# TAMS-Group/bio_ik

Measured on AMD Instinct MI355X. Metric: IK solves/sec (pop=128, 7-DOF PoseGoal batch), higher is better.
Workload: dtype f64

## Files before the change

bio_ik_amd/csrc/bioik_kernels.h:

```cpp
#pragma once
#include <type_traits>

#include "bioik_device.h"


#ifndef BIOIK_CANDIDATE_BOUND
#define BIOIK_CANDIDATE_BOUND BIOIK_SINCOS_DOMAIN
#endif
#ifndef BIOIK_COOP_WALKS
#define BIOIK_COOP_WALKS 1
#endif

struct LdsLayout {
    int seed, par, pop, sol, prefix, state, clip, xcol, slots, g_first, g_stride, total;
    int xn, gv, frames, tips, delta, base, grad, red, sec, order, bc;
    int xm, xp, dv, fc;
    int fitp;
    int help;
};
BIOIK_HD LdsLayout make_layout(int n_ops, int V, int P, int T, int n_slots, int nthreads, int lambda, int has_secondary, int child_cols = 1,
                               int groups = 1, int slot_sets = 1, int fit_park = 0, int fc_in_pop = 0, int helped = 0, int bounded = 0) {
    LdsLayout L;
    const int m = n_ops > 0 ? n_ops : 1;
    int o = 0;
// ... 62 lines not shown
};
BIOIK_DEV bool cand_better(double f, int pos, double of, int opos) { return (f < of) || (f == of && pos < opos); }

BIOIK_DEV void top2_insert(double& b1f, int& b1p, double& b2f, int& b2p, double f, int pos) {
    const bool w1 = cand_better(f, pos, b1f, b1p), w2 = cand_better(f, pos, b2f, b2p);
    b2f = w1 ? b1f : (w2 ? f : b2f);
    b2p = w1 ? b1p : (w2 ? pos : b2p);
    b1f = w1 ? f : b1f;
    b1p = w1 ? pos : b1p;
}
BIOIK_DEV void top2_merge(double& b1f, int& b1p, double& b2f, int& b2p, double o1f, int o1p, double o2f, int o2p) {
    const bool w1 = cand_better(o1f, o1p, b1f, b1p);
    const bool k2 = cand_better(b1f, b1p, o2f, o2p);
    const bool w2 = cand_better(o1f, o1p, b2f, b2p);
    const double n2f = w1 ? (k2 ? b1f : o2f) : (w2 ? o1f : b2f);
    const int n2p = w1 ? (k2 ? b1p : o2p) : (w2 ? o1p : b2p);
    b1f = w1 ? o1f : b1f;
    b1p = w1 ? o1p : b1p;
    b2f = n2f, b2p = n2p;
}
BIOIK_DEV double wave_min_f64(double v) {
    v = fmin(v, p_quad_xor<1>(v));
    v = fmin(v, p_quad_xor<2>(v));
    v = fmin(v, p_row_mirror<1>(v));
    v = fmin(v, p_row_mirror<0>(v));
    return fmin(fmin(p_read_lane(v, 0), p_read_lane(v, 16)), fmin(p_read_lane(v, 32), p_read_lane(v, 48)));
}
BIOIK_DEV int imin(int a, int b) { return a < b ? a : b; }
BIOIK_DEV int wave_min_i32(int v) {
    v = imin(v, p_quad_xor<1>(v));
    v = imin(v, p_quad_xor<2>(v));
    v = imin(v, p_row_mirror<1>(v));
    v = imin(v, p_row_mirror<0>(v));
    return imin(imin(p_read_lane(v, 0), p_read_lane(v, 16)), imin(p_read_lane(v, 32), p_read_lane(v, 48)));
}
BIOIK_DEV int wave_argmin(double f, int pos, double& mf, int& mp) {
    mf = wave_min_f64(f);
    const unsigned long long tied = p_ballot(f == mf);
    int lane;
    if ((tied & (tied - 1ull)) == 0ull) {
        lane = __builtin_ctzll(tied);
    } else {
        const int pm = wave_min_i32(f == mf ? pos : 0x7fffffff);
        lane = __builtin_ctzll(p_ballot(f == mf && pos == pm));
    }
    mp = p_read_lane(pos, lane);
    return lane;
}
BIOIK_DEV void top2_wave64_minima(double& b1f, int& b1p, double& b2f, int& b2p) {
    double w1f, w2f;
    int w1p, w2p;
    const int l1 = wave_argmin(b1f, b1p, w1f, w1p);
    const bool mine = (p_tid() & 63) == l1;
    wave_argmin(mine ? b2f : b1f, mine ? b2p : b1p, w2f, w2p);
    b1f = w1f, b1p = w1p, b2f = w2f, b2p = w2p;
}
BIOIK_DEV void top2_wave(double& b1f, int& b1p, double& b2f, int& b2p, int G) {
#if !defined(BIOIK_TOP2_BUTTERFLY)
    if (G >= 64) {
        top2_wave64_minima(b1f, b1p, b2f, b2p);
        return;
    }
#endif
#pragma unroll
    for (int m = 32; m >= 16; m >>= 1) {
        if (m >= G) continue;
        double o1f = p_shfl_xor(b1f, m), o2f = p_shfl_xor(b2f, m);
        int o1p = p_shfl_xor(b1p, m), o2p = p_shfl_xor(b2p, m);
        top2_merge(b1f, b1p, b2f, b2p, o1f, o1p, o2f, o2p);
    }
#define TOP2_DPP_STEP(MOVE)                                          \
    {                                                                \
        const double o1f = MOVE(b1f), o2f = MOVE(b2f);               \
        const int o1p = MOVE(b1p), o2p = MOVE(b2p);                  \
        top2_merge(b1f, b1p, b2f, b2p, o1f, o1p, o2f, o2p);          \
    }
    TOP2_DPP_STEP(p_row_mirror<0>)
    TOP2_DPP_STEP(p_row_mirror<1>)
    TOP2_DPP_STEP(p_quad_xor<2>)
    TOP2_DPP_STEP(p_quad_xor<1>)
#undef TOP2_DPP_STEP
}
template <int E>
BIOIK_DEV void sort_pairs_in_registers(double (&f)[E], int (&c)[E], int gtid, int G) {
    const int n = G * E;
    for (int k = 2; k <= n; k <<= 1) {
        const bool ascending = ((gtid * E) & k) == 0;
        for (int j = k >> 1; j >= E; j >>= 1) {
            const int d = j / E;
            const bool keep_low = ((gtid & d) == 0) == ascending;
#pragma unroll
            for (int i = 0; i < E; i++) {
                const double of = p_shfl_xor(f[i], d);
                const int oc = p_shfl_xor(c[i], d);
                const bool mine_after = (f[i] > of) || (f[i] == of && c[i] > oc);
                const bool take = mine_after == keep_low;
                f[i] = take ? of : f[i], c[i] = take ? oc : c[i];
            }
        }
#pragma unroll
        for (int j = E >> 1; j > 0; j >>= 1) {
            if (j >= k) continue;
#pragma unroll
            for (int i = 0; i < E; i++) {
                if (i & j) continue;
                const int i2 = i | j;
                const bool asc = k >= E ? ascending : ((i & k) == 0);
                const bool a_after_b = (f[i] > f[i2]) || (f[i] == f[i2] && c[i] > c[i2]);
                const bool swap = a_after_b == asc;
                const double fa = f[i], fb = f[i2];
                const int ca = c[i], cb = c[i2];
                f[i] = swap ? fb : fa, f[i2] = swap ? fa : fb, c[i] = swap ? cb : ca, c[i2] = swap ? ca : cb;
            }
        }
    }
}
template <int E>
BIOIK_DEV void sort_keys_in_registers(unsigned long long (&key)[E], int gtid, int G) {
    const int n = G * E;
    for (int k = 2; k <= n; k <<= 1) {
        const bool ascending = ((gtid * E) & k) == 0;
        for (int j = k >> 1; j >= E; j >>= 1) {
            const int d = j / E;
            const bool keep_low = ((gtid & d) == 0) == ascending;
#pragma unroll
            for (int i = 0; i < E; i++) {
                const unsigned long long other = p_shfl_xor(key[i], d);
                key[i] = ((key[i] > other) == keep_low) ? other : key[i];
            }
        }
#pragma unroll
        for (int j = E >> 1; j > 0; j >>= 1) {
            if (j >= k) continue;
#pragma unroll
            for (int i = 0; i < E; i++) {
                if (i & j) continue;
                const int i2 = i | j;
                const bool asc = k >= E ? ascending : ((i & k) == 0);
                const unsigned long long a = key[i], b = key[i2];
                const bool swap = (a > b) == asc;
                key[i] = swap ? b : a, key[i2] = swap ? a : b;
            }
        }
    }
}
BIOIK_DEV unsigned long long half_min_u64(unsigned long long k) {
    unsigned long long o = p_shfl_xor(k, 16);
    k = o < k ? o : k;
    o = p_row_mirror<0>(k), k = o < k ? o : k;
    o = p_row_mirror<1>(k), k = o < k ? o : k;
    o = p_quad_xor<2>(k), k = o < k ? o : k;
    o = p_quad_xor<1>(k), k = o < k ? o : k;
    return k;
}
BIOIK_DEV unsigned long long group_min_u64(unsigned long long k, int G) {
    if (G >= 64) {
        const unsigned long long o = p_shfl_xor(k, 32);
        k = o < k ? o : k;
    }
    return half_min_u64(k);
}
template <int E>
BIOIK_DEV unsigned long long select_threshold(const unsigned long long (&key)[E], int n_mine, int k, int G, unsigned long long gmask, bool& found) {
    unsigned long long lo = ~0ull, nhi = ~0ull;
#pragma unroll
    for (int i = 0; i < E; i++)
        if (i < n_mine) lo = key[i] < lo ? key[i] : lo, nhi = ~key[i] < nhi ? ~key[i] : nhi;
    lo = group_min_u64(lo, G);
    unsigned long long hi = ~group_min_u64(nhi, G);
    unsigned long long T = hi;
    bool done = false;
    for (int round = 0; round < 66; round++) {
        const unsigned long long mid = lo + ((hi - lo) >> 1);
        int cnt = 0;
#pragma unroll
        for (int i = 0; i < E; i++) cnt += p_popc64(p_ballot(key[i] <= mid) & gmask);
        if (!done) {
            if (cnt == k) T = mid, done = true;
            else if (cnt < k) lo = mid + 1ull;
            else hi = mid;
        }
        if (p_ballot(!done) == 0ull) break;
    }
    found = done;
    return T;
}
BIOIK_DEV unsigned long long sort_key(double f, int index, int drop) {
    unsigned long long b;
    __builtin_memcpy(&b, &f, 8);
    return (b & ~((1ull << drop) - 1ull)) | (unsigned long long)index;
}
BIOIK_DEV void group_sync(int G) {
    if (G > 64) p_barrier(); else p_wave_sync();
}
BIOIK_DEV void top2_xwave(double& b1f, int& b1p, double& b2f, int& b2p, double* s_red, int gtid, int G) {
    const int nw = G >> 6;
    if (G > 64) {
        if ((gtid & 63) == 0) {
            double* d = s_red + 4 * (gtid >> 6);
            d[0] = b1f, d[1] = (double)b1p, d[2] = b2f, d[3] = (double)b2p;
        }
        p_barrier();
        b1f = b2f = P_INF;
        b1p = b2p = 0x7fffffff;
        for (int w = 0; w < nw; w++) {
            const double* d = s_red + 4 * w;
            for (int i = 0; i < 2; i++) {
                double of = d[2 * i];
                int op = (int)d[2 * i + 1];
                top2_insert(b1f, b1p, b2f, b2p, of, op);
            }
        }
        p_barrier();
    }
}

template <int COOP = 0, class PB>
BIOIK_NOINLINE void build_approximator(PB pb, XV x, double* slots, double* s_frames, double* s_tips, double* s_delta, double* s_base, int gtid, int G,
                                       const double* prefix = nullptr) {
    const int n_ops = pb->n_ops, T = pb->T;
    if (gtid < 64) {
        auto publish = [&](int t, const F7& f) {
            if (gtid == 0) f7_store(s_tips + t * 7, f);
        };
        if (COOP == 0) fk_walk(pb, x, slots, gtid == 0 ? s_frames : nullptr, publish, prefix);
        else if (G >= 64) fk_walk<64>(pb, x, slots, gtid == 0 ? s_frames : nullptr, publish, prefix);
        else fk_walk<32>(pb, x, slots, gtid == 0 ? s_frames : nullptr, publish, prefix);
    }
    for (int k = gtid; k < n_ops; k += G) s_base[k] = x(k);
    group_sync(G);
    for (int t = 0; t < T; t++)
        for (int k = gtid; k < n_ops; k += G) {
            double o[7];
            approximator_entry(pb, t, k, s_frames, s_tips, o, s_base, prefix);
            double* d = s_delta + ((size_t)t * n_ops + k) * 7;
            for (int c = 0; c < 7; c++) d[c] = o[c];
        }
    group_sync(G);
}

struct SelectArgs {
    int islands, V;
    int sync, pad;
    uint64_t n;
    const double* isl_solutions;
    const double* isl_fitness;
    const int32_t* isl_success;
    const int32_t* isl_steps;
    double* solutions;
    double* fitness;
    int32_t* success;
    int32_t* steps;
};
BIOIK_DEV void select_body(const SelectArgs& a, uint64_t q) {
    if (q >= a.n) return;
    int best = 0;
    double best_fit = BIOIK_DBL_MAX;
    int least_steps = 0x7fffffff;
    if (a.sync)
        for (int i = 0; i < a.islands; i++) {
            uint64_t u = q * (uint64_t)a.islands + i;
            if (p_load_device(a.isl_success + u) && p_load_device(a.isl_steps + u) < least_steps) least_steps = p_load_device(a.isl_steps + u);
        }
    for (int i = 0; i < a.islands; i++) {
        uint64_t u = q * (uint64_t)a.islands + i;
        if (p_load_device(a.isl_success + u) && (!a.sync || p_load_device(a.isl_steps + u) == least_steps) && p_load_device(a.isl_fitness + u) < best_fit) best_fit = p_load_device(a.isl_fitness + u), best = i;
    }
    if (best_fit == BIOIK_DBL_MAX) {
        for (int i = 0; i < a.islands; i++) {
            uint64_t u = q * (uint64_t)a.islands + i;
            if (p_load_device(a.isl_fitness + u) < best_fit) best_fit = p_load_device(a.isl_fitness + u), best = i;
        }
    }
    uint64_t u = q * (uint64_t)a.islands + best;
    for (int v = 0; v < a.V; v++) a.solutions[q * a.V + v] = p_load_device(a.isl_solutions + u * a.V + v);
    a.fitness[q] = best_fit;
    a.success[q] = p_load_device(a.isl_success + u);
    a.steps[q] = p_load_device(a.isl_steps + u);
}

BIOIK_DEV void select_coop(const SelectArgs& a, uint64_t q, int lane) {
    const uint64_t u0 = q * (uint64_t)a.islands;
    int least = 0x7fffffff;
    if (a.sync) {
        for (int i = lane; i < a.islands; i += 64) {
            const int st = p_load_device(a.isl_steps + u0 + i);
            if (p_load_device(a.isl_success + u0 + i) && st < least) least = st;
        }
        for (int m = 32; m >= 1; m >>= 1) {
            const int o = p_shfl_xor(least, m);
            least = o < least ? o : least;
        }
    }
    double bf = BIOIK_DBL_MAX, af = BIOIK_DBL_MAX;
    int bi = 0x7fffffff, ai = 0x7fffffff;
    for (int i = lane; i < a.islands; i += 64) {
        const double f = p_load_device(a.isl_fitness + u0 + i);
        const bool counts = p_load_device(a.isl_success + u0 + i) && (!a.sync || p_load_device(a.isl_steps + u0 + i) == least);
        if (counts && f < bf) bf = f, bi = i;
        if (f < af) af = f, ai = i;
    }
    for (int m = 32; m >= 1; m >>= 1) {
        const double obf = p_shfl_xor(bf, m), oaf = p_shfl_xor(af, m);
        const int obi = p_shfl_xor(bi, m), oai = p_shfl_xor(ai, m);
        if (obf < bf || (obf == bf && obi < bi)) bf = obf, bi = obi;
        if (oaf < af || (oaf == af && oai < ai)) af = oaf, ai = oai;
// ... 720 lines not shown
template <class Frame>
BIOIK_DEV void solve_walks(Frame& F, SpeciesState& S, double*& popS, int rank_it, int step, int gen, uint32_t ctr1, int n_eval, double& b1f, int& b1p, double& b2f, int& b2p) {
    BIOIK_FRAME_NAMES(F);
    auto rank_now = [&]() { return F.rank_now(rank_it); };
    unsigned int& gen_count = F.gen_count;
    bool& lost = F.lost;
    auto rendezvous_lost = [&]() { F.rendezvous_lost(); };
    BIOIK_LANE_SCOPE;
    const double* cb = popS + S.cur * BF;
    const double *p0g = cb, *p0d = cb + M, *p1d = cb + 3 * M;
    const uint32_t gctr = (uint32_t)step * 16u + (uint32_t)gen;
    const bool stored = !columnless && n_cols * G >= lambda && (LEAN || pb->n_quat == 0);
    auto offer = [&](double f, int pos) { top2_insert(b1f, b1p, b2f, b2p, f, pos); };
    auto coarse_parked = [&](int gt) {
        if constexpr (SLIM && CL) {
            if (const int tie_bits = a.preselect >> 8) {
                double* const s_fq = gbase + L.fitp;
                for (int r = gt; r < n_eval; r += G) {
                    unsigned long long v;
                    __builtin_memcpy(&v, &s_fq[r], 8);
                    v &= ~((1ull << tie_bits) - 1ull);
                    __builtin_memcpy(&s_fq[r], &v, 8);
                }
                group_sync(G);
            }
        }
    };
    if (!JOINT && stored && child_pairs && exact) {
        for (int r = gtid, j = 0; r < n_eval; r += 2 * G, j += 2) {
            const int r1 = r + G;
            const bool two = r1 < n_eval;
            const int c0 = has_sec ? s_order[r] : r;
            const int c1 = two ? (has_sec ? s_order[r1] : r1) : c0;
            double* const xc[2] = {xcol + (size_t)j * M * nth, two ? xcol + (size_t)(j + 1) * M * nth : xcol + (size_t)j * M * nth};
            const uint32_t ci[2] = {(uint32_t)c0 + 2u, (uint32_t)c1 + 2u};
            reproduce_children<2>(pb, key, ctr1, ci, p0g, p0d, p1d, xc, nth);
            PHASE_MARK(PH_REPRODUCE);
            const XV xv[2] = {XV{xc[0], nth}, XV{xc[1], nth}};
            double f[2];
            eval_exact_primary_n<2>(pb, xv, qc, s_slots, pb->n_slots * 7 * nth, f, s_prefix);
            PHASE_MARK(PH_FITNESS);
            offer(f[0], r + 2);
            if (two) offer(f[1], r1 + 2);
        }
    } else if (JOINT) {
        if constexpr (JOINT) {
            const int cb_off = (int)(cb - lds);
            const int cbo[2] = {p_read_lane(cb_off, 0), p_read_lane(cb_off, 32)};
            const int ob_off = (int)(popS + (S.cur ^ 1) * BF - lds);
            const int obo[2] = {p_read_lane(ob_off, 0), p_read_lane(ob_off, 32)};
            const int ct[2] = {p_read_lane((int)ctr1, 0), p_read_lane((int)ctr1, 32)};
            const int ne0 = p_read_lane(n_eval, 0), total = ne0 + p_read_lane(n_eval, 32);
            if constexpr (SLIM) {
                for (int t0 = 0; t0 < total; t0 += 128) {
                    double f[2];
                    {
                        BIOIK_LANE_SCOPE;
                        const int i0r = t0 + tid, i0 = i0r < total ? i0r : 0, i1 = i0r + 64 < total ? i0r + 64 : i0;
                        const int sp0 = i0 >= ne0 ? 1 : 0, sp1 = i1 >= ne0 ? 1 : 0;
                        const int r0 = i0 - (sp0 ? ne0 : 0), r1 = i1 - (sp1 ? ne0 : 0);
                        const int32_t* const ord0 = (const int32_t*)(lds + L.g_first + L.order);
                        const int c0 = ord0[sp0 * 2 * L.g_stride + r0], c1 = ord0[sp1 * 2 * L.g_stride + r1];
                        const double *pa = lds + (sp0 ? cbo[1] : cbo[0]), *pc = lds + (sp1 ? cbo[1] : cbo[0]);
                        const ChildT<PB> cx[2] = {make_child_t(pb, key, (uint32_t)(sp0 ? ct[1] : ct[0]), (uint32_t)c0 + 2u, pa, lds + (sp0 ? obo[1] : obo[0]), M),
                                                  make_child_t(pb, key, (uint32_t)(sp1 ? ct[1] : ct[0]), (uint32_t)c1 + 2u, pc, lds + (sp1 ? obo[1] : obo[0]), M)};
                        PHASE_MARK(PH_REPRODUCE);
                        eval_exact_primary_n<2, true>(pb, cx, qc, s_slots, pb->n_slots * 7 * nth, f, s_prefix);
                        PHASE_MARK(PH_FITNESS);
                    }
                    BIOIK_LANE_SCOPE;
                    const int i0r = t0 + tid, i0 = i0r < total ? i0r : 0, i1 = i0r + 64 < total ? i0r + 64 : i0;
                    const int sp0 = i0 >= ne0 ? 1 : 0, sp1 = i1 >= ne0 ? 1 : 0;
                    const int r0 = i0 - (sp0 ? ne0 : 0), r1 = i1 - (sp1 ? ne0 : 0);
                    if (pb->n_link_primary < pb->n_primary) {
                        const int32_t* const ord0 = (const int32_t*)(lds + L.g_first + L.order);
                        const int c0 = ord0[sp0 * 2 * L.g_stride + r0], c1 = ord0[sp1 * 2 * L.g_stride + r1];
                        const double *pa = lds + (sp0 ? cbo[1] : cbo[0]), *pc = lds + (sp1 ? cbo[1] : cbo[0]);
                        const ChildX<PB> cx[2] = {make_child_x(pb, key, (uint32_t)(sp0 ? ct[1] : ct[0]), (uint32_t)c0 + 2u, pa, pa + M, pa + 3 * M),
                                                  make_child_x(pb, key, (uint32_t)(sp1 ? ct[1] : ct[0]), (uint32_t)c1 + 2u, pc, pc + M, pc + 3 * M)};
                        f[0] = nonlink_primary(pb, cx[0], qc, f[0]), f[1] = nonlink_primary(pb, cx[1], qc, f[1]);
                    } else {
                        f[0] += 0.0, f[1] += 0.0;
                    }
                    f[0] += balance_cost(pb, v3(0.0, 0.0, 0.0), qc), f[1] += balance_cost(pb, v3(0.0, 0.0, 0.0), qc);
                    if (i0r < total) (lds + L.g_first + sp0 * L.g_stride + L.fitp)[r0] = f[0];
                    if (i0r + 64 < total) (lds + L.g_first + sp1 * L.g_stride + L.fitp)[r1] = f[1];
                }
                p_wave_sync();
            }
        }
    } else if (!JOINT && columnless && child_pairs && exact) {
        if constexpr (HELPED) {
            unsigned int* const hw = (unsigned int*)(lds + L.help);
            {
                BIOIK_LANE_SCOPE;
                const int w = p_wave_index();
                if (gtid == 0) {
                    hw[6 + 4 * w] = (unsigned int)(int)(p0g - lds), hw[7 + 4 * w] = (unsigned int)(int)(popS + (S.cur ^ 1) * BF - lds);
                    hw[8 + 4 * w] = ctr1, hw[9 + 4 * w] = (unsigned int)n_eval;
                }
                p_wave_sync();
                gen_count++;
                p_flag_store(hw + 2 + w, gen_count);
            }
            for (int r0 = 0; r0 < n_eval; r0 += 128) {
                double f[1];
                {
                    BIOIK_LANE_SCOPE;
                    const int r = r0 + gtid, ra = r < n_eval ? r : 0;
                    const int c = has_sec ? s_order[ra] : ra;
                    const uint32_t ctr1t = rng_ctr1(gctr, (uint32_t)species_load(rank_now()).id, RNG_REPRODUCE);
                    const double* const pgt = popS + (S.cur ^ 1) * BF;
                    const ChildT<PB> cx[1] = {make_child_t(pb, key, ctr1t, (uint32_t)c + 2u, p0g, pgt, M)};
                    PHASE_MARK(PH_REPRODUCE);
                    eval_exact_primary_n<1, true, true>(pb, cx, qc, s_slots, 0, f, s_prefix);
                }
                BIOIK_LANE_SCOPE;
                const int r = r0 + gtid;
                if (pb->n_link_primary < pb->n_primary) {
                    const SpeciesState S2 = species_load(rank_now());
                    const double* cb2 = s_pop + S2.slot * SP + S2.cur * BF;
                    const uint32_t ctr2 = rng_ctr1(gctr, (uint32_t)S2.id, RNG_REPRODUCE);
                    const int ra2 = r < n_eval ? r : 0;
                    f[0] = nonlink_primary(pb, make_child_x(pb, key, ctr2, (uint32_t)(has_sec ? s_order[ra2] : ra2) + 2u, cb2, cb2 + M, cb2 + 3 * M), qc, f[0]);
                } else {
                    f[0] += 0.0;
                }
                f[0] += balance_cost(pb, v3(0.0, 0.0, 0.0), qc);
                PHASE_MARK(PH_FITNESS);
                double* const s_fit = gbase + L.fitp;
                if (r < n_eval) s_fit[r] = f[0];
            }
            {
                BIOIK_LANE_SCOPE;
                p_wave_sync();
                if (!lost && p_flag_wait_ge(hw + 4 + p_wave_index(), gen_count) == 0xffffffffu) rendezvous_lost();
            }
            {
                BIOIK_LANE_SCOPE;
                const double* const s_fit2 = gbase + L.fitp;
                coarse_parked(gtid);
                for (int r = gtid; r < n_eval; r += G) offer(s_fit2[r], r + 2);
            }
        } else if constexpr (SLIM) {
            for (int r0 = 0; r0 < n_eval; r0 += 2 * G) {
                double f[2];
                {
                    BIOIK_LANE_SCOPE;
                    const int r = r0 + gtid, r1 = r + G;
                    const bool two = r1 < n_eval;
                    const int ra = r < n_eval ? r : 0, rb = two ? r1 : ra;
                    const int c0 = has_sec ? s_order[ra] : ra, c1 = has_sec ? s_order[rb] : rb;
                    const uint32_t ctr1t = rng_ctr1(gctr, (uint32_t)species_load(rank_now()).id, RNG_REPRODUCE);
                    if constexpr (DENSE || WAVE2) {
                        const double* const pgt = popS + (S.cur ^ 1) * BF;
                        const ChildT<PB> cx[2] = {make_child_t(pb, key, ctr1t, (uint32_t)c0 + 2u, p0g, pgt, M), make_child_t(pb, key, ctr1t, (uint32_t)c1 + 2u, p0g, pgt, M)};
                        PHASE_MARK(PH_REPRODUCE);
                        eval_exact_primary_n<2, true, true>(pb, cx, qc, s_slots, 0, f, s_prefix);
                    } else {
                        const ChildX<PB> cx[2] = {make_child_x(pb, key, ctr1t, (uint32_t)c0 + 2u, p0g, p0d, p1d), make_child_x(pb, key, ctr1t, (uint32_t)c1 + 2u, p0g, p0d, p1d)};
                        PHASE_MARK(PH_REPRODUCE);
                        eval_exact_primary_n<2, true, FIXED != 0>(pb, cx, qc, s_slots, pb->n_slots * 7 * nth, f, s_prefix);
                    }
                }
                BIOIK_LANE_SCOPE;
                const int r = r0 + gtid, r1 = r + G;
                const bool two = r1 < n_eval;
                if (pb->n_link_primary < pb->n_primary) {
                    const SpeciesState S2 = species_load(rank_now());
                    const double* cb2 = s_pop + S2.slot * SP + S2.cur * BF;
                    const uint32_t ctr2 = rng_ctr1(gctr, (uint32_t)S2.id, RNG_REPRODUCE);
                    const int ra = r < n_eval ? r : 0, rb = two ? r1 : ra;
                    const int c0 = has_sec ? s_order[ra] : ra, c1 = has_sec ? s_order[rb] : rb;
                    const ChildX<PB> cx[2] = {make_child_x(pb, key, ctr2, (uint32_t)c0 + 2u, cb2, cb2 + M, cb2 + 3 * M),
                                              make_child_x(pb, key, ctr2, (uint32_t)c1 + 2u, cb2, cb2 + M, cb2 + 3 * M)};
                    f[0] = nonlink_primary(pb, cx[0], qc, f[0]), f[1] = nonlink_primary(pb, cx[1], qc, f[1]);
                } else {
                    f[0] += 0.0, f[1] += 0.0;
                }
                f[0] += balance_cost(pb, v3(0.0, 0.0, 0.0), qc), f[1] += balance_cost(pb, v3(0.0, 0.0, 0.0), qc);
                PHASE_MARK(PH_FITNESS);
                double* const s_fit = gbase + L.fitp;
                if (r < n_eval) s_fit[r] = f[0];
                if (two) s_fit[r1] = f[1];
            }
            if constexpr (!DENSE) {
                BIOIK_LANE_SCOPE;
                const double* const s_fit2 = gbase + L.fitp;
                coarse_parked(gtid);
                for (int r = gtid; r < n_eval; r += G) offer(s_fit2[r], r + 2);
            }
        } else
        for (int r = gtid; r < n_eval; r += 2 * G) {
            const int r1 = r + G;
            const bool two = r1 < n_eval;
            const int c0 = has_sec ? s_order[r] : r;
            const int c1 = two ? (has_sec ? s_order[r1] : r1) : c0;
            const ChildX<PB> cx[2] = {make_child_x(pb, key, ctr1, (uint32_t)c0 + 2u, p0g, p0d, p1d),
                                      make_child_x(pb, key, ctr1, (uint32_t)c1 + 2u, p0g, p0d, p1d)};
            PHASE_MARK(PH_REPRODUCE);
            double f[2];
            eval_exact_primary_n<2>(pb, cx, qc, s_slots, pb->n_slots * 7 * nth, f, s_prefix);
            PHASE_MARK(PH_FITNESS);
            offer(f[0], r + 2);
            if (two) offer(f[1], r1 + 2);
        }
    } else if (!JOINT && columnless) {
        for (int r = gtid; r < n_eval; r += G) {
            const int c = has_sec ? s_order[r] : r;
            const auto cx = make_child_x(pb, key, ctr1, (uint32_t)c + 2u, p0g, p0d, p1d);
            PHASE_MARK(PH_REPRODUCE);
            const double f = exact ? eval_exact_primary(pb, cx, qc, s_slots, s_prefix) : eval_linear_primary(pb, cx, qc, lm);
            PHASE_MARK(PH_FITNESS);
            offer(f, r + 2);
        }
    } else {
        for (int r = gtid, j = 0; r < n_eval; r += G, j++) {
            int c = has_sec ? s_order[r] : r;
            double* xc = stored ? xcol + (size_t)j * M * nth : xcol;
            const XV xv{xc, nth};
            reproduce_child(pb, key, ctr1, (uint32_t)c + 2u, p0g, p0d, p1d, xc, nth, nullptr, 0);
            PHASE_MARK(PH_REPRODUCE);
            double f = exact ? eval_exact_primary(pb, xv, qc, s_slots, s_prefix) : eval_linear_primary(pb, xv, qc, lm);
            PHASE_MARK(PH_FITNESS);
            offer(f, r + 2);
        }
    }
}

template <class Frame>
BIOIK_DEV void solve_select_and_copy(Frame& F, SpeciesState& S, double*& popS, int rank_it, int step, int gen, uint32_t ctr1, int n_eval, double& b1f, int& b1p, double& b2f, int& b2p) {
    BIOIK_FRAME_NAMES(F);
    auto rank_now = [&]() { return F.rank_now(rank_it); };
    BIOIK_LANE_SCOPE;
    const double* cb = popS + S.cur * BF;
    const double *p0g = cb, *p0d = cb + M, *p1d = cb + 3 * M;
    const bool stored = !columnless && n_cols * G >= lambda && (LEAN || pb->n_quat == 0);
    auto offer = [&](double f, int pos) { top2_insert(b1f, b1p, b2f, b2p, f, pos); };
    auto coarse_parked = [&](int gt) {
        if constexpr (SLIM && CL) {
            if (const int tie_bits = a.preselect >> 8) {
                double* const s_fq = gbase + L.fitp;
                for (int r = gt; r < n_eval; r += G) {
                    unsigned long long v;
                    __builtin_memcpy(&v, &s_fq[r], 8);
                    v &= ~((1ull << tie_bits) - 1ull);
                    __builtin_memcpy(&s_fq[r], &v, 8);
                }
                group_sync(G);
            }
        }
    };
    if constexpr (SLIM) S = species_load(rank_now()), popS = s_pop + S.slot * SP, cb = popS + S.cur * BF, p0g = cb, p0d = cb + M, p1d = cb + 3 * M;
    const uint32_t ctr1w = SLIM ? rng_ctr1((uint32_t)step * 16u + (uint32_t)gen, (uint32_t)S.id, RNG_REPRODUCE) : ctr1;
    if constexpr (DENSE || JH) coarse_parked(gtid);
    if constexpr (DENSE || JH) {
        const double* const s_fit2 = gbase + L.fitp;
        const int drop = a.sort_key_drop;
        unsigned long long k1 = ~0ull, k2 = ~0ull;
        for (int r = gtid; r < n_eval; r += G) {
            const unsigned long long k = sort_key(s_fit2[r], r + 2, drop);
            const bool w1 = k < k1, w2 = k < k2;
            k2 = w1 ? k1 : (w2 ? k : k2);
            k1 = w1 ? k : k1;
        }
        const unsigned long long B1 = half_min_u64(k1);
        const unsigned long long B2 = half_min_u64(k1 == B1 ? k2 : k1);
        int shares = 0;
        for (int r = gtid; r < n_eval; r += G) shares += ((sort_key(s_fit2[r], r + 2, drop) ^ B2) >> drop) == 0ull ? 1 : 0;
        const unsigned long long one = p_ballot(shares > 0), more = p_ballot(shares > 1);
        const uint32_t mine = grp ? (uint32_t)(one >> 32) : (uint32_t)one;
        const bool in_doubt = B2 != ~0ull && ((mine & (mine - 1u)) != 0u);
        if (p_ballot(in_doubt) == 0ull && more == 0ull) {
            b1p = (int)(B1 & 1023ull), b1f = s_fit2[b1p - 2];
            if (B2 != ~0ull) b2p = (int)(B2 & 1023ull), b2f = s_fit2[b2p - 2];
        } else {
            for (int r = gtid; r < n_eval; r += G) offer(s_fit2[r], r + 2);
            top2_wave(b1f, b1p, b2f, b2p, G);
        }
    } else {
        top2_wave(b1f, b1p, b2f, b2p, G);
    }
    PHASE_MARK(PH_SEL_TOP2);
    top2_xwave(b1f, b1p, b2f, b2p, s_red, gtid, G);
    PHASE_MARK(PH_SEL_XWAVE);
    if constexpr (SELECTS) {
        if (has_sec) {
            double* const s_fv = gbase + L.fitp;
            int t1 = 0, t2 = 0;
            for (int r = gtid; r < n_eval; r += G) {
                const double v = s_fv[r];
                t1 += v == b1f ? 1 : 0, t2 += v == b2f ? 1 : 0;
            }
            const unsigned long long gm = G >= 64 ? ~0ull : 0xffffffffull << (tid & 32);
            const unsigned long long o1 = p_ballot(t1 > 0) & gm, o2 = p_ballot(t2 > 0) & gm;
            const bool tie = (p_ballot(t1 > 1 || t2 > 1) & gm) != 0ull || (o1 & (o1 - 1ull)) != 0ull || (o2 & (o2 - 1ull)) != 0ull || (b2p != 0x7fffffff && b2f == S.pf0);
            if (p_ballot(tie) != 0ull) {
                auto stable_first = [&](double fwant, int skip, double& wf, int& wc) -> int {
                    double bs = P_INF;
                    int bc = 0x7fffffff, br = 0x7fffffff;
                    for (int r = gtid; r < n_eval; r += G) {
                        if (!(s_fv[r] == fwant) || r == skip) continue;
                        const int c = s_order[r];
                        const double sec = secondary_fitness<true>(pb, make_child_x(pb, key, ctr1w, (uint32_t)c + 2u, p0g, p0d, p1d), qc);
                        if (sec < bs || (sec == bs && c < bc)) bs = sec, bc = c, br = r;
                    }
                    double w2f = P_INF;
                    int w2c = 0x7fffffff;
                    wf = bs, wc = bc;
                    top2_wave(wf, wc, w2f, w2c, G);
                    const unsigned long long own = p_ballot(bc == wc && bc != 0x7fffffff) & gm;
                    const int src = own != 0ull ? __builtin_ctzll(own) : (tid & 63);
                    const int rr = p_shfl(br, src);
                    return own != 0ull ? rr : 0x7fffffff;
                };
                double e1, e2;
                int c1, c2;
                const int r1 = stable_first(b1f, -1, e1, c1);
                const int r2 = stable_first(b2f, r1, e2, c2);
                if (tie && r1 != 0x7fffffff) {
                    b1p = r1 + 2;
                    if (b2p != 0x7fffffff && r2 != 0x7fffffff) {
                        b2p = r2 + 2;
                        const bool first_is_first = e1 < e2 || (e1 == e2 && c1 < c2);
                        if (first_is_first != (r1 < r2)) {
                            if (gtid == 0) {
                                const int ca = s_order[r1], cb2 = s_order[r2];
                                const double fa = s_fv[r1], fb = s_fv[r2];
                                s_order[r1] = cb2, s_order[r2] = ca, s_fv[r1] = fb, s_fv[r2] = fa;
                            }
                            b1p = r2 + 2, b2p = r1 + 2;
                        }
                    }
                }
                group_sync(G);
            }
        }
    }
    Cand first{S.pf0, 0, 0};
    if (cand_better(S.pf1, 1, first.f, first.pos)) first = Cand{S.pf1, 1, 1};
    if (cand_better(b1f, b1p, first.f, first.pos)) first = Cand{b1f, b1p, b1p};
    const double c2f = (b1p == first.id) ? b2f : b1f;
    const int c2p = (b1p == first.id) ? b2p : b1p;
    Cand second{P_INF, 0x7fffffff, -1};
    if (first.id != 0) second = Cand{S.pf0, first.pos, 0};
    if (first.id != 1 && (second.id < 0 || cand_better(S.pf1, 1, second.f, second.pos))) second = Cand{S.pf1, 1, 1};
    if (second.id < 0 || cand_better(c2f, c2p, second.f, second.pos)) second = Cand{c2f, c2p, c2p};
    double* nb = popS + (S.cur ^ 1) * BF;
    const bool both_at_once = G >= 64 || M <= 16;
    for (int pass = 0; pass < (both_at_once ? 1 : 2); pass++) {
        BIOIK_LANE_SCOPE;
        if (gtid >= 64) break;
        const int i = G >= 64 ? gtid >> 5 : (both_at_once ? gtid >> 4 : pass), k0 = G >= 64 || !both_at_once ? gtid & 31 : gtid & 15;
        const int id = i == 0 ? first.id : second.id;
        double* dst = nb + i * 2 * M;
        if (id < 2) {
            const double* src = cb + id * 2 * M;
            if (k0 < M) dst[k0] = src[k0], dst[M + k0] = src[M + k0];
            if (M > 32 && k0 + 32 < M) dst[k0 + 32] = src[k0 + 32], dst[M + k0 + 32] = src[M + k0 + 32];
        } else if (stored) {
            BIOIK_FP_STRICT
            const int r = id - 2;
            const int c = has_sec ? s_order[r] : r;
            const double fmix = (((uint32_t)c + 2u) % 2u == 0u) ? 0.2 : 0.0;
            const int r_col = (G & (G - 1)) == 0 ? r >> (31 - __builtin_clz((unsigned)G)) : r / G, r_lane = r - r_col * G;
            const double* src = (lds + L.xcol) + (size_t)r_col * M * nth + (grp * G + r_lane);
            auto take = [&](int k) {
                double gene = src[(size_t)k * nth];
                double mom = 0.0;
                if ((active_mask >> k) & 1ull) {
                    double parent_gradient = p0d[k] * (1.0 - fmix) + p1d[k] * fmix;
                    mom = parent_gradient * (1.0 - 0.3) + (gene - p0g[k]) * 0.3;
                }
                dst[k] = gene, dst[M + k] = mom;
            };
            if (k0 < n_ops) take(k0);
            if (n_ops > 32 && k0 + 32 < n_ops) take(k0 + 32);
        } else if (LEAN) {
            BIOIK_FP_STRICT
            const int c = has_sec ? s_order[id - 2] : id - 2;
            const ChildX<PB> cx = make_child_x(pb, key, ctr1w, (uint32_t)c + 2u, p0g, p0d, p1d);
            auto derive = [&](int k) {
                const double gene = cx.template value<false>(k);
                double mom = 0.0;
                if ((active_mask >> k) & 1ull) {
                    const double parent_gradient = p0d[k] * (1.0 - cx.fmix) + p1d[k] * cx.fmix;
                    mom = parent_gradient * (1.0 - 0.3) + (gene - p0g[k]) * 0.3;
                }
                dst[k] = gene, dst[M + k] = mom;
            };
            if (k0 < n_ops) derive(k0);
            if (n_ops > 32 && k0 + 32 < n_ops) derive(k0 + 32);
        } else if (k0 == 0) {
            int c = has_sec ? s_order[id - 2] : id - 2;
            reproduce_child(pb, key, ctr1, (uint32_t)c + 2u, p0g, p0d, p1d, dst, 1, dst + M, 1);
        }
    }
    S.cur ^= 1;
    S.pf0 = first.f;
    S.pf1 = second.f;
    if constexpr (SLIM)
        if (gtid == 0) species_store(rank_now(), S);
    group_sync(G);
    PHASE_MARK(PH_SEL_COPY);
    group_sync(G);
    PHASE_MARK(PH_SEL_BAR);
}

template <class Frame>
BIOIK_DEV void solve_generation(Frame& F, SpeciesState& S, double*& popS, int rank_it, int step, int gen) {
    BIOIK_FRAME_NAMES(F);
    auto rank_now = [&]() { return F.rank_now(rank_it); };
    BIOIK_LANE_SCOPE;
    if constexpr (SLIM) S = species_load(rank_now()), popS = s_pop + S.slot * SP;
    const double* cb = popS + S.cur * BF;
    const double *p0g = cb, *p0d = cb + M, *p1d = cb + 3 * M;
    const uint32_t gctr = (uint32_t)step * 16u + (uint32_t)gen;
    const uint32_t ctr1 = rng_ctr1(gctr, (uint32_t)S.id, RNG_REPRODUCE);
    int n_eval = lambda;
    uint64_t inside_mask = 0ull;
    if constexpr (DENSE || WAVE2 || JH) {
        double* const pgt = popS + (S.cur ^ 1) * BF;
        bool inside = false;
        for (int k = gtid; k < n_ops; k += G) {
            const double d0 = p0d[k], d1 = p1d[k];
            const double pg0 = child_parent_gradient(d0, d1, 0), pg1 = child_parent_gradient(d0, d1, 1);
            pgt[k] = pg0, pgt[M + k] = pg1;
            if constexpr (WAVE2)
                inside = pb->ops[k].gene >= 0 && !op_unbounded(pb, k) && avoid_limits_surely_free(p0g[k], pg0, pg1, op_limit<LIM_VMIN>(pb, k), op_limit<LIM_VMAX>(pb, k), op_limit<LIM_SPAN>(pb, k));
        }
        if constexpr (WAVE2) inside_mask = has_sec ? p_ballot(inside) : 0ull;
        group_sync(G);
    }
    if (has_sec) solve_preselect(F, S, popS, step, gen, ctr1, inside_mask, n_eval);
    double b1f = P_INF, b2f = P_INF;
    int b1p = 0x7fffffff, b2p = 0x7fffffff;
    solve_walks(F, S, popS, rank_it, step, gen, ctr1, n_eval, b1f, b1p, b2f, b2p);
    solve_select_and_copy(F, S, popS, rank_it, step, gen, ctr1, n_eval, b1f, b1p, b2f, b2p);
}

template <class Frame>
BIOIK_DEV void solve_memetic(Frame& F, SpeciesState& S, double*& popS, int rank_it, int step) {
    BIOIK_FRAME_NAMES(F);
    auto rank_now = [&]() { return F.rank_now(rank_it); };
    if constexpr (SLIM) S = species_load(rank_now()), popS = s_pop + S.slot * SP;
    if (sp.memetic) {
        BIOIK_LANE_SCOPE;
        double* el = popS + S.cur * BF;
        const XV xe{el, 1};
        if (exact) build_approximator<BIOIK_COOP_WALKS>(pb, xe, s_slots, s_frames, s_tips, s_delta, s_base, gtid, G, s_prefix);
        PHASE_MARK(PH_MEM_APPROX);
        if (gtid < 64) {
            const int Gw = G < 64 ? G : 64;
            double dp = 0.0000001;
            {
                uint32_t o0, o1;
                philox2x32_10(key, rng_ctr0(0, 0), rng_ctr1((uint32_t)step * 16u, (uint32_t)S.id, RNG_MEMETIC_SIGN), o0, o1);
                if (rng_uniform(o0, o1) < 0.5) dp = -dp;
            }
            const bool by_op = pb_flavour<PB>::general ? pb->genes_follow_ops != 0 : true;
            const int cnt = by_op ? n_ops : D;
            const int my_op = gtid < D ? pb->op_of_gene[gtid] : -1;
            double* s_gop = s_gv;
            const int FB = 8 * T;
            double* s_x4 = s_xn;
            double* s_ex = s_bc;
            auto chains = [&](const double* d0, double* f0, const double* d1, double* f1) {
                for (int idx = gtid; idx < FB; idx += Gw) {
                    const int t = idx >> 3, c = idx & 7;
                    if (c == 7) continue;
                    double a0 = s_tips[t * 7 + c], a1 = a0;
                    const double* dl = s_delta + (size_t)t * n_ops * 7 + c;
                    for (int g0 = 0; g0 < cnt; g0 += 4) {
                        double d[4], v0[4], v1[4];
#pragma unroll
                        for (int j = 0; j < 4; j++) {
                            const int i2 = g0 + j < cnt ? g0 + j : cnt - 1;
                            const int kk = by_op ? i2 : pb->op_of_gene[i2];
                            const bool pad = g0 + j >= cnt;
                            d[j] = dl[(size_t)kk * 7];
                            v0[j] = pad ? 0.0 : d0[kk];
                            v1[j] = (pad || !d1) ? 0.0 : d1[kk];
                        }
#pragma unroll
                        for (int j = 0; j < 4; j++) {
                            a0 = BK_FMA(d[j], v0[j], a0);
                            if (d1) a1 = BK_FMA(d[j], v1[j], a1);
                        }
                    }
                    f0[idx] = a0;
                    if (d1) f1[idx] = a1;
                }
            };
            auto frame_of = [&](const double* fc, int t) { return f7_load(fc + t * 8); };
            double* const s_tm = s_dv;
            auto secondary_shared = [&](const PerturbX& xown, const PerturbX& x, const double* tm) -> double {
                double sum = 0.0;
                const F7 zero = F7{{0.0, 0.0, 0.0}, {0.0, 0.0, 0.0, 0.0}};
                for (int g = 0; g < pb->n_secondary; g++) {
                    const int type = pb->secondary[g].type;
                    double e;
                    if (joint_set_is_sum(type)) {
                        p_wave_sync();
                        for (int k = gtid; k < n_ops; k += Gw) {
                            s_tm[k] = joint_set_term(pb, type, k, x.el[k], qc.seed);
                            if (x.el2) s_tm[3 * M + k] = joint_set_term(pb, type, k, x.el2[k], qc.seed);
                        }
                        p_wave_sync();
                        const double own = x.op >= 0 ? joint_set_term(pb, type, x.op, x.el[x.op] + x.step, qc.seed) : 0.0;
                        e = 0.0;
                        if (by_op) {
                            for (int k = 0; k < n_ops; k++) e += k == x.op ? own : tm[k];
                        } else {
                            for (int i = 0; i < D; i++) {
                                const int k = pb->op_of_gene[i];
                                e += k == x.op ? own : tm[k];
                            }
                        }
                    } else {
                        e = goal_eval<false, PerturbX>(pb, type, pb->secondary[g].var_op, pb->secondary[g].var_seed, qc.par + pb->secondary[g].param_off, zero, xown, qc, pb->secondary[g].pad);
                    }
                    sum += e * pb->secondary[g].weight_sq;
                }
                return sum;
            };
            auto goals_on = [&](const double* fc, int dop, double dstep, const PerturbX& x, double& prim, double& all, bool want_all, const PerturbX& xsh, const double* tm) {
#if !defined(BIOIK_NO_POSE_ONLY)
                if (pb->pose_only) {
                    F7 f = frame_of(fc, 0);
                    if (dstep != 0.0 && dop >= 0) {
                        const double* dl = s_delta + (size_t)dop * 7;
                        f = F7{{BK_FMA(dl[0], dstep, f.p.x), BK_FMA(dl[1], dstep, f.p.y), BK_FMA(dl[2], dstep, f.p.z)},
                               {BK_FMA(dl[3], dstep, f.q.x), BK_FMA(dl[4], dstep, f.q.y), BK_FMA(dl[5], dstep, f.q.z), BK_FMA(dl[6], dstep, f.q.w)}};
                    }
                    const double* P = qc.par + pb->pose_param_off;
                    double e = dist2(f.p, v3(P[0], P[1], P[2]));
                    const Q4 d = Q4{P[3] - f.q.x, P[4] - f.q.y, P[5] - f.q.z, P[6] - f.q.w};
                    const Q4 a = Q4{P[3] + f.q.x, P[4] + f.q.y, P[5] + f.q.z, P[6] + f.q.w};
                    const double rs = P[7];
                    e += fmin(qdot(d, d), qdot(a, a)) * (rs * rs);
                    prim = all = e * pb->pose_weight_sq;
                    return;
                }
#endif
                double acc = 0.0;
                V3 bal = v3(0.0, 0.0, 0.0);
                auto tip_frame = [&](int t) -> F7 {
                    F7 f = frame_of(fc, t);
                    if (dstep != 0.0) {
                        double d[7] = {0.0, 0.0, 0.0, 0.0, 0.0, 0.0, 0.0};
                        if (dop >= 0) {
                            const double* dl = s_delta + ((size_t)t * n_ops + dop) * 7;
                            for (int c = 0; c < 7; c++) d[c] = dl[c];
                        }
                        f = F7{{BK_FMA(d[0], dstep, f.p.x), BK_FMA(d[1], dstep, f.p.y), BK_FMA(d[2], dstep, f.p.z)},
                               {BK_FMA(d[3], dstep, f.q.x), BK_FMA(d[4], dstep, f.q.y), BK_FMA(d[5], dstep, f.q.z), BK_FMA(d[6], dstep, f.q.w)}};
                    }
                    return f;
                };
                for (int t = 0; t < T; t++) {
                    const F7 f = tip_frame(t);
                    acc = tip_goals(pb, t, f, x, qc, acc, tip_frame);
                    balance_tip(pb, t, f, bal);
                }
                acc = nonlink_primary(pb, x, qc, acc);
                acc += balance_cost(pb, bal, qc);
                prim = acc;
                if constexpr (DENSE) all = acc + 0.0;
                else all = want_all ? acc + secondary_shared(x, xsh, tm) : acc;
            };
            if constexpr (DENSE) {
                const bool in0 = gtid < n_ops, wide = n_ops > 32, in1 = wide && gtid + 32 < n_ops;
                const int k1 = gtid + 32;
                const bool on0 = in0 && ((active_mask >> gtid) & 1ull), on1 = in1 && ((active_mask >> k1) & 1ull);
                const double base0 = in0 ? s_base[gtid] : 0.0, cmin0 = in0 ? s_clip[gtid] : 0.0, cmax0 = in0 ? s_clip[M + gtid] : 0.0;
                double e0 = in0 ? el[gtid] : 0.0;
                double* const fcb = L.fc >= 0 ? s_fc : popS + (S.cur ^ 1) * BF;
                const int n4 = n_ops & ~3;
                const bool comp0 = gtid < FB && (gtid & 7) != 7;
                const double tip0 = comp0 ? s_tips[(gtid >> 3) * 7 + (gtid & 7)] : 0.0;
                const double* const dl0 = s_delta + ((gtid >> 3) * n_ops * 7 + (gtid & 7));
                auto chain_of = [&](auto two, const double start, const double* dl, const double* u, double* out) {
                    constexpr bool TWO = decltype(two)::value;
                    const double* w = u + M;
// ... 651 lines not shown
```

Measured before the change: 1.298 million.

## Specialize DENSE path: shared RNG stream, tournament top-2 keys, regenerate winners on copy

For the DENSE variant, the per-generation RNG child stream is computed once by lane 0, stored in s_red, and reused when building children, which avoids rehashing the key and counter per child. Top-2 selection now loads a fixed unrolled set of keys per lane, runs a register tournament and does the wave reduction on 32-bit words, and counts ties with ballots. The winner copy recomputes the winning child's genes and momentum from the RNG stream instead of reading stored columns. This cuts RNG and reduction overhead but duplicates the mutation math, so it depends on bit-exact agreement with the evaluated children.

```diff
diff --git a/bio_ik_amd/csrc/bioik_kernels.h b/bio_ik_amd/csrc/bioik_kernels.h
--- a/bio_ik_amd/csrc/bioik_kernels.h
+++ b/bio_ik_amd/csrc/bioik_kernels.h
@@ -238,6 +238,51 @@
     o = p_quad_xor<2>(k), k = o < k ? o : k;
     o = p_quad_xor<1>(k), k = o < k ? o : k;
     return k;
+}
+template <int N>
+BIOIK_DEV void top2_of_keys(const unsigned long long (&k)[N], unsigned long long& k1, unsigned long long& k2) {
+    static_assert(N >= 2 && (N & (N - 1)) == 0, "a tournament over a power of two of keys");
+    unsigned long long a[N / 2], b[N / 2];
+#pragma unroll
+    for (int i = 0; i < N / 2; i++) {
+        const bool w = k[2 * i + 1] < k[2 * i];
+        a[i] = w ? k[2 * i + 1] : k[2 * i], b[i] = w ? k[2 * i] : k[2 * i + 1];
+    }
+#pragma unroll
+    for (int n = N / 2; n > 1; n >>= 1) {
+#pragma unroll
+        for (int i = 0; i < n / 2; i++) {
+            const bool w = a[2 * i + 1] < a[2 * i];
+            const unsigned long long lead = w ? a[2 * i + 1] : a[2 * i], other = w ? a[2 * i] : a[2 * i + 1], second = w ? b[2 * i + 1] : b[2 * i];
+            a[i] = lead, b[i] = second < other ? second : other;
+        }
+    }
+    k1 = a[0], k2 = b[0];
+}
+BIOIK_DEV uint32_t dense_stream_word(const double* s_red) { return *(const uint32_t*)s_red; }
+template <class PB>
+BIOIK_DEV ChildT<PB> child_t_of_stream(PB pb, uint32_t stream, uint32_t child_index, const double* p0g, const double* pgtable, int M) {
+    ChildT<PB> c;
+    c.pb = pb, c.p0g = p0g;
+    c.pgrow = pgtable + (int)(child_index % 2u) * M;
+    c.base = rng_child_base(stream, child_index);
+    c.mutation_rate = rng_child_rate(c.base);
+    c.gradient_factor = (double)(child_index % 3u);
+    return c;
+}
+BIOIK_DEV uint32_t half_min_u32(uint32_t v) {
+    uint32_t o = (uint32_t)p_shfl_xor((int)v, 16);
+    v = o < v ? o : v;
+    o = (uint32_t)p_row_mirror<0>((int)v), v = o < v ? o : v;
+    o = (uint32_t)p_row_mirror<1>((int)v), v = o < v ? o : v;
+    o = (uint32_t)p_quad_xor<2>((int)v), v = o < v ? o : v;
+    o = (uint32_t)p_quad_xor<1>((int)v), v = o < v ? o : v;
+    return v;
+}
+BIOIK_DEV unsigned long long half_min_u64_by_words(unsigned long long k) {
+    const uint32_t hi = (uint32_t)(k >> 32), least_hi = half_min_u32(hi);
+    const uint32_t least_lo = half_min_u32(hi == least_hi ? (uint32_t)k : 0xffffffffu);
+    return ((unsigned long long)least_hi << 32) | least_lo;
 }
 BIOIK_DEV unsigned long long group_min_u64(unsigned long long k, int G) {
     if (G >= 64) {
@@ -1264,7 +1309,13 @@
                     const int ra = r < n_eval ? r : 0, rb = two ? r1 : ra;
                     const int c0 = has_sec ? s_order[ra] : ra, c1 = has_sec ? s_order[rb] : rb;
                     const uint32_t ctr1t = rng_ctr1(gctr, (uint32_t)species_load(rank_now()).id, RNG_REPRODUCE);
-                    if constexpr (DENSE || WAVE2) {
+                    if constexpr (DENSE) {
+                        const double* const pgt = popS + (S.cur ^ 1) * BF;
+                        const uint32_t stream = dense_stream_word(s_red);
+                        const ChildT<PB> cx[2] = {child_t_of_stream(pb, stream, (uint32_t)c0 + 2u, p0g, pgt, M), child_t_of_stream(pb, stream, (uint32_t)c1 + 2u, p0g, pgt, M)};
+                        PHASE_MARK(PH_REPRODUCE);
+                        eval_exact_primary_n<2, true, true>(pb, cx, qc, s_slots, 0, f, s_prefix);
+                    } else if constexpr (WAVE2) {
                         const double* const pgt = popS + (S.cur ^ 1) * BF;
                         const ChildT<PB> cx[2] = {make_child_t(pb, key, ctr1t, (uint32_t)c0 + 2u, p0g, pgt, M), make_child_t(pb, key, ctr1t, (uint32_t)c1 + 2u, p0g, pgt, M)};
                         PHASE_MARK(PH_REPRODUCE);
@@ -1366,7 +1417,47 @@
     if constexpr (SLIM) S = species_load(rank_now()), popS = s_pop + S.slot * SP, cb = popS + S.cur * BF, p0g = cb, p0d = cb + M, p1d = cb + 3 * M;
     const uint32_t ctr1w = SLIM ? rng_ctr1((uint32_t)step * 16u + (uint32_t)gen, (uint32_t)S.id, RNG_REPRODUCE) : ctr1;
     if constexpr (DENSE || JH) coarse_parked(gtid);
-    if constexpr (DENSE || JH) {
+    if constexpr (DENSE) {
+        const double* const s_fit2 = gbase + L.fitp;
+        const int drop = a.sort_key_drop;
+        const unsigned long long low = (1ull << drop) - 1ull;
+        const uint32_t keep_lo = (uint32_t)~low, keep_hi = (uint32_t)(~low >> 32);
+        unsigned long long B1, B2, one = 0ull, more = 0ull;
+        auto by_keys = [&](auto n_keys) {
+            constexpr int NK = decltype(n_keys)::value;
+            unsigned long long k[NK];
+            bool held[NK];
+#pragma unroll
+            for (int i = 0; i < NK; i++) {
+                const int r = gtid + 32 * i;
+                held[i] = i < 4 || r < n_eval;
+                unsigned long long b;
+                __builtin_memcpy(&b, &s_fit2[held[i] ? r : gtid], 8);
+                const uint32_t lo = ((uint32_t)b & keep_lo) | (uint32_t)(r + 2), hi = (uint32_t)(b >> 32) & keep_hi;
+                k[i] = held[i] ? ((unsigned long long)hi << 32) | lo : ~0ull;
+            }
+            unsigned long long k1, k2;
+            top2_of_keys<NK>(k, k1, k2);
+            B1 = half_min_u64_by_words(k1);
+            B2 = half_min_u64_by_words(k1 == B1 ? k2 : k1);
+#pragma unroll
+            for (int i = 0; i < NK; i++) {
+                const unsigned long long m = p_ballot(held[i] && (k[i] ^ B2) <= low);
+                more |= one & m, one |= m;
+            }
+        };
+        if (n_eval <= 128) by_keys(std::integral_constant<int, 4>{});
+        else by_keys(std::integral_constant<int, 8>{});
+        const uint32_t mine = grp ? (uint32_t)(one >> 32) : (uint32_t)one;
+        const bool in_doubt = B2 != ~0ull && ((mine & (mine - 1u)) != 0u);
+        if (p_ballot(in_doubt) == 0ull && more == 0ull) {
+            b1p = (int)(B1 & 1023ull), b1f = s_fit2[b1p - 2];
+            if (B2 != ~0ull) b2p = (int)(B2 & 1023ull), b2f = s_fit2[b2p - 2];
+        } else {
+            for (int r = gtid; r < n_eval; r += G) offer(s_fit2[r], r + 2);
+            top2_wave(b1f, b1p, b2f, b2p, G);
+        }
+    } else if constexpr (JH) {
         const double* const s_fit2 = gbase + L.fitp;
         const int drop = a.sort_key_drop;
         unsigned long long k1 = ~0ull, k2 = ~0ull;
@@ -1460,6 +1551,53 @@
     if (second.id < 0 || cand_better(c2f, c2p, second.f, second.pos)) second = Cand{c2f, c2p, c2p};
     double* nb = popS + (S.cur ^ 1) * BF;
     const bool both_at_once = G >= 64 || M <= 16;
+    if constexpr (DENSE) {
+        const double* const pgt = nb;
+        for (int pass = 0; pass < (both_at_once ? 1 : 2); pass++) {
+            BIOIK_LANE_SCOPE;
+            const int i = both_at_once ? gtid >> 4 : 1 - pass, k0 = both_at_once ? gtid & 15 : gtid;
+            const int id = i == 0 ? first.id : second.id;
+            double* dst = nb + i * 2 * M;
+            double v[2][2] = {{0.0, 0.0}, {0.0, 0.0}};
+            const bool wide = n_ops > 32;
+            if (id < 2) {
+                const double* src = cb + id * 2 * M;
+                if (k0 < M) v[0][0] = src[k0], v[0][1] = src[M + k0];
+                if (wide && k0 + 32 < M) v[1][0] = src[k0 + 32], v[1][1] = src[M + k0 + 32];
+            } else {
+                BIOIK_FP_STRICT
+                const uint32_t child = (uint32_t)(id - 2) + 2u;
+                const ChildT<PB> cx = child_t_of_stream(pb, dense_stream_word(s_red), child, p0g, pgt, M);
+                auto derive = [&](int k, double (&o)[2]) {
+                    const double parent_gene = p0g[k], parent_gradient = cx.pgrow[k];
+                    const int g = pb->ops[k].gene;
+                    double gene = parent_gene, mom = 0.0;
+                    if (g >= 0) {
+                        const uint32_t word = rng_child_word(cx.base, (uint32_t)(g + 1));
+                        const double r = rng_gauss32(word);
+                        const double f = cx.mutation_rate * op_limit<LIM_SPAN>(pb, k);
+                        double gn = parent_gene;
+                        gn += r * f;
+                        const double g2 = parent_gradient * cx.gradient_factor;
+                        gn += g2;
+                        gene = p_clamp(gn, s_clip[k], s_clip[M + k]);
+                        mom = parent_gradient * (1.0 - 0.3) + (gene - parent_gene) * 0.3;
+                    }
+                    o[0] = gene, o[1] = mom;
+                };
+                if (k0 < n_ops) derive(k0, v[0]);
+                if (wide && k0 + 32 < n_ops) derive(k0 + 32, v[1]);
+            }
+            p_wave_sync();
+            if (id < 2) {
+                if (k0 < M) dst[k0] = v[0][0], dst[M + k0] = v[0][1];
+                if (wide && k0 + 32 < M) dst[k0 + 32] = v[1][0], dst[M + k0 + 32] = v[1][1];
+            } else {
+                if (k0 < n_ops) dst[k0] = v[0][0], dst[M + k0] = v[0][1];
+                if (wide && k0 + 32 < n_ops) dst[k0 + 32] = v[1][0], dst[M + k0 + 32] = v[1][1];
+            }
+        }
+    } else
     for (int pass = 0; pass < (both_at_once ? 1 : 2); pass++) {
         BIOIK_LANE_SCOPE;
         if (gtid >= 64) break;
@@ -1542,6 +1680,8 @@
                 inside = pb->ops[k].gene >= 0 && !op_unbounded(pb, k) && avoid_limits_surely_free(p0g[k], pg0, pg1, op_limit<LIM_VMIN>(pb, k), op_limit<LIM_VMAX>(pb, k), op_limit<LIM_SPAN>(pb, k));
         }
         if constexpr (WAVE2) inside_mask = has_sec ? p_ballot(inside) : 0ull;
+        if constexpr (DENSE)
+            if (gtid == 0) *(uint32_t*)s_red = rng_child_stream(key, ctr1);
         group_sync(G);
     }
     if (has_sec) solve_preselect(F, S, popS, step, gen, ctr1, inside_mask, n_eval);
```

Measured after the change: 1.330 million, median of 6. +2.5%, better.
